# vaenyr/stable-diffusion-on-device

Measured on AMD Instinct MI355X. Metric: images/sec + per-UNet-step ms, SD v1.4 512x512 20-step PLMS, 1/2/4/8 MI355X, higher is better.
Workload: dtype f16

## Files before the change

stable-diffusion-on-device_amd/csrc/attention.hip:

```cpp
#include "common.h"
#include "sdod_hip.h"
#include "host_util.h"

#include <cstdlib>
#include <type_traits>

namespace {

struct AttnP {
    const f16* q;
    const f16* k;
    const f16* v;
    f16* out;
    int B, H, Lq, Lk;
    int ldq, ldk, ldv, ldo;
    float scale_log2;
    int causal;
};

typedef short short4v __attribute__((__vector_size__(4 * sizeof(short))));
typedef __attribute__((address_space(3))) short4v* lds_short4_ptr;

constexpr int odd16(int dv) {
    int s = (dv + 15) / 16;
    if ((s & 1) == 0) s += 1;
    return s * 16;
}

template <int D, int QT>
constexpr int attn_min_waves() { return (D == 40 || (D == 80 && QT == 1)) ? 3 : 1; }

template <int N, int I = 0, class F>
SDOD_DEVICE void static_for(F&& f) {
    if constexpr (I < N) {
        f(std::integral_constant<int, I>{});
        static_for<N, I + 1>(f);
    }
}

template <int D, int QT, bool TR, int KVS = 1>
__global__ __launch_bounds__(256 * KVS, (attn_min_waves<D, QT>())) void attn_kernel(const AttnP p) {
    constexpr int DP = ((D + 31) / 32) * 32;
    constexpr int KSTEPS = DP / 32;
    constexpr int DV = ((D + 15) / 16) * 16;
    constexpr int NDT = DV / 16;
    constexpr int KSTR = DP + 8;
    constexpr int VSTR = odd16(DV);
    constexpr int KT = 64;
    constexpr int DC = D / 8;
    constexpr int LD_IT = (KT * DC + 255) / 256;
    constexpr int STAGE = KT * (KSTR + VSTR);
    constexpr bool SUM_BY_MFMA = DV > D;
    static_assert(D % 8 == 0, "head dim must be a multiple of 8");

    extern __shared__ __attribute__((aligned(16))) char smem_raw[];
    const int grp = KVS > 1 ? (int)(threadIdx.x >> 8) : 0;
    f16* smem = reinterpret_cast<f16*>(smem_raw) + (size_t)grp * 2 * STAGE;

    const int tid = threadIdx.x & 255;
    const int lane = tid & 63;
    const int wave = tid >> 6;
    const int g = lane >> 4;
    const int li = lane & 15;
    const int nqb = (p.Lq + 64 * QT - 1) / (64 * QT);
    const int lid = xcd_remap(blockIdx.x, nqb * p.H * p.B);
    const int bh = lid / nqb;
    const int b = bh / p.H, h = bh - b * p.H;
    const int q_block = (lid - bh * nqb) * (64 * QT);

    const f16* kbase = p.k + (size_t)b * p.Lk * p.ldk + h * D;
    const f16* vbase = p.v + (size_t)b * p.Lk * p.ldv + h * D;

    {
        constexpr int KPADC = (DP - D) / 8, VPADC = (DV - D) / 8;
        for (int st = 0; st < 2; ++st) {
            f16* sK = smem + st * STAGE;
            f16* sV = sK + KT * KSTR;
            if (KPADC > 0)
                for (int idx = tid; idx < KT * KPADC; idx += 256) {
                    const int row = idx / (KPADC > 0 ? KPADC : 1), ch = idx - row * KPADC;
                    *reinterpret_cast<f16x8*>(sK + row * KSTR + D + ch * 8) = zero8();
                }
            if (VPADC > 0)
                for (int idx = tid; idx < KT * VPADC; idx += 256) {
                    const int row = idx / (VPADC > 0 ? VPADC : 1), ch = idx - row * VPADC;
                    f16x8 pad = zero8();
                    if (ch == 0) pad[0] = (f16)1.0f;
                    *reinterpret_cast<f16x8*>(sV + row * VSTR + D + ch * 8) = pad;
                }
        }
    }

    f16x8 qf[QT][KSTEPS];
    int qrow[QT];
#pragma unroll
    for (int t = 0; t < QT; ++t) {
        qrow[t] = q_block + wave * (16 * QT) + t * 16 + li;
        const f16* qp = p.q + ((size_t)b * p.Lq + qrow[t]) * p.ldq + h * D;
#pragma unroll
        for (int ks = 0; ks < KSTEPS; ++ks) {
            const int d0 = ks * 32 + g * 8;
            qf[t][ks] = (qrow[t] < p.Lq && d0 + 8 <= D) ? ldg8(qp + d0) : zero8();
        }
    }

    int kend = p.Lk;
    if (p.causal) kend = min(p.Lk, q_block + 64 * QT);
    const int NT = (kend + KT - 1) / KT;

    f16x8 rk[LD_IT], rv[LD_IT];
    const f16* kptr0[LD_IT];
    const f16* vptr0[LD_IT];
#pragma unroll
    for (int i = 0; i < LD_IT; ++i) {
        const int idx = tid + 256 * i;
        const int row = idx / DC, ch = idx - row * DC;
        kptr0[i] = kbase + (size_t)row * p.ldk + ch * 8;
        vptr0[i] = vbase + (size_t)row * p.ldv + ch * 8;
    }
    auto load_tile = [&](int t) {
        if (t * KT + KT <= p.Lk) {
            const size_t ko = (size_t)t * KT * p.ldk, vo = (size_t)t * KT * p.ldv;
#pragma unroll
            for (int i = 0; i < LD_IT; ++i) {
                if (tid + 256 * i < KT * DC) {
                    rk[i] = ldg8(kptr0[i] + ko);
                    rv[i] = ldg8(vptr0[i] + vo);
                }
            }
            return;
        }
#pragma unroll
        for (int i = 0; i < LD_IT; ++i) {
            const int idx = tid + 256 * i;
            const int row = idx / DC, ch = idx - row * DC;
            const int key = t * KT + row;
            const bool ok = (idx < KT * DC) && (key < p.Lk);
            rk[i] = ok ? ldg8(kbase + (size_t)key * p.ldk + ch * 8) : zero8();
            rv[i] = ok ? ldg8(vbase + (size_t)key * p.ldv + ch * 8) : zero8();
        }
    };
    auto store_tile = [&](int st) {
        f16* sK = smem + st * STAGE;
        f16* sV = sK + KT * KSTR;
#pragma unroll
        for (int i = 0; i < LD_IT; ++i) {
            const int idx = tid + 256 * i;
            const int row = idx / DC, ch = idx - row * DC;
            if (idx < KT * DC) {
                *reinterpret_cast<f16x8*>(sK + row * KSTR + ch * 8) = rk[i];
                *reinterpret_cast<f16x8*>(sV + row * VSTR + ch * 8) = rv[i];
            }
        }
    };

    f32x4 o[QT][NDT];
    float m_run[QT], l_run[QT];
#pragma unroll
    for (int t = 0; t < QT; ++t) {
        m_run[t] = -1e30f;
        l_run[t] = 0.f;
#pragma unroll
        for (int dt = 0; dt < NDT; ++dt) o[t][dt] = f32x4{0.f, 0.f, 0.f, 0.f};
    }

#ifdef SDOD_ATTN_ABLATE
    constexpr int abl = SDOD_ATTN_ABLATE;
#else
    constexpr int abl = 0;
#endif
    constexpr bool HOLD = D <= 80;
    auto read_vt = [&](const f16* sV, int u, int dt) -> f16x8 {
        const f16* a0 = sV + (32 * u + 4 * g + (li >> 2)) * VSTR + dt * 16 + 4 * (li & 3);
        const short4v lo = __builtin_amdgcn_ds_read_tr16_b64_v4i16((lds_short4_ptr)(a0));
        const short4v hi = __builtin_amdgcn_ds_read_tr16_b64_v4i16((lds_short4_ptr)(a0 + 16 * VSTR));
        typedef short short8v __attribute__((__vector_size__(8 * sizeof(short))));
        const short8v both = __builtin_shufflevector(lo, hi, 0, 1, 2, 3, 4, 5, 6, 7);
        return __builtin_bit_cast(f16x8, both);
    };
    auto softmax_pv = [&](auto a_c, int t, f32x4 (&s_a)[4], const f16x8 (&vfr)[HOLD ? 2 : 1][HOLD ? NDT : 1], const f16* sV) {
        constexpr int a = decltype(a_c)::value;
        const bool need_mask = (t * KT + KT > p.Lk) || (p.causal && (t * KT + KT - 1 > q_block + wave * (16 * QT)));
        if (need_mask) {
            int key0 = t * KT + g * 4;
            asm volatile("" : "+v"(key0));
#pragma unroll
            for (int c = 0; c < 4; ++c)
#pragma unroll
                for (int r = 0; r < 4; ++r) {
                    const int key = key0 + c * 16 + r;
                    const bool masked = (key >= p.Lk) | (p.causal & (key > qrow[a]));
                    s_a[c][r] = masked ? -1e30f : s_a[c][r];
                }
        }
        float mx;
        {
            const float t0 = fmaxf(fmaxf(s_a[0][0], s_a[0][1]), s_a[0][2]);
            const float t1 = fmaxf(fmaxf(s_a[0][3], s_a[1][0]), s_a[1][1]);
            const float t2 = fmaxf(fmaxf(s_a[1][2], s_a[1][3]), s_a[2][0]);
            const float t3 = fmaxf(fmaxf(s_a[2][1], s_a[2][2]), s_a[2][3]);
            const float t4 = fmaxf(fmaxf(s_a[3][0], s_a[3][1]), s_a[3][2]);
            const float u0 = fmaxf(fmaxf(t0, t1), t2);
            const float u1 = fmaxf(fmaxf(t3, t4), s_a[3][3]);
            mx = fmaxf(u0, u1);
        }
        mx = quad_rows_max(mx);
        const float m_new = fmaxf(m_run[a], mx * p.scale_log2);
        const bool rescale = __builtin_amdgcn_ballot_w64(m_new != m_run[a]) != 0;
        const float alpha = rescale ? __builtin_amdgcn_exp2f(m_run[a] - m_new) : 1.0f;
        m_run[a] = m_new;
        float rs[4] = {0.f, 0.f, 0.f, 0.f};
        const float sc = p.scale_log2, nm = -m_new;
#pragma unroll
        for (int c = 0; c < 4; ++c) {
#pragma unroll
            for (int r = 0; r < 4; ++r) {
                float v = __builtin_fmaf(s_a[c][r], sc, nm);
                if (!(abl & 2)) v = __builtin_amdgcn_exp2f(v);
                if (!SUM_BY_MFMA) rs[r] += v;
                s_a[c][r] = v;
            }
        }
        if (!SUM_BY_MFMA) l_run[a] = __builtin_fmaf(l_run[a], alpha, (rs[0] + rs[1]) + (rs[2] + rs[3]));
        if (rescale) {
#pragma unroll
            for (int dt = 0; dt < NDT; ++dt)
#pragma unroll
                for (int r = 0; r < 4; ++r) o[a][dt][r] *= alpha;
        }
        f16x8 pf[2];
#pragma unroll
        for (int u = 0; u < 2; ++u) {
            f16x8 f;
#pragma unroll
            for (int r = 0; r < 4; ++r) {
                f[r] = (f16)s_a[2 * u][r];
                f[4 + r] = (f16)s_a[2 * u + 1][r];
            }
            pf[u] = f;
        }
#pragma unroll
        for (int u = 0; u < 2; ++u) {
#pragma unroll
            for (int dt = 0; dt < NDT; ++dt) {
                f16x8 vf;
                if (TR) {
                    vf = HOLD ? vfr[u][dt] : read_vt(sV, u, dt);
                } else {
#pragma unroll
                    for (int e = 0; e < 8; ++e) vf[e] = sV[(32 * u + 16 * (e >> 2) + 4 * g + (e & 3)) * VSTR + dt * 16 + li];
                }
                o[a][dt] = mfma16(vf, pf[u], o[a][dt]);
            }
        }
    };
    auto read_k = [&](const f16* sK, f16x8 (&kf)[HOLD ? KSTEPS : 1][4]) {
        if constexpr (HOLD) {
#pragma unroll
            for (int ks = 0; ks < KSTEPS; ++ks)
#pragma unroll
                for (int c = 0; c < 4; ++c) kf[ks][c] = *reinterpret_cast<const f16x8*>(sK + (c * 16 + li) * KSTR + ks * 32 + g * 8);
        }
    };
    auto read_v = [&](const f16* sV, f16x8 (&vfr)[HOLD ? 2 : 1][HOLD ? NDT : 1]) {
        if constexpr (TR && HOLD) {
#pragma unroll
            for (int u = 0; u < 2; ++u)
#pragma unroll
                for (int dt = 0; dt < NDT; ++dt) vfr[u][dt] = read_vt(sV, u, dt);
        }
    };
    auto qk = [&](const f16* sK, const f16x8 (&kf)[HOLD ? KSTEPS : 1][4], f32x4 (&s)[QT][4]) {
#pragma unroll
        for (int a = 0; a < QT; ++a) {
#pragma unroll
            for (int c = 0; c < 4; ++c) s[a][c] = f32x4{0.f, 0.f, 0.f, 0.f};
#pragma unroll
            for (int ks = 0; ks < KSTEPS; ++ks)
#pragma unroll
                for (int c = 0; c < 4; ++c) {
                    const f16x8 k8 = HOLD ? kf[ks][c] : *reinterpret_cast<const f16x8*>(sK + (c * 16 + li) * KSTR + ks * 32 + g * 8);
                    s[a][c] = mfma16(k8, qf[a][ks], s[a][c]);
                }
        }
    };

    if (grp < NT) {
        load_tile(grp);
        store_tile(0);
    }
    __syncthreads();
    const int NTG = (NT + KVS - 1) / KVS;
    for (int it = 0; it < NTG; ++it) {
        const int t = it * KVS + grp;
        const int cur = it & 1;
        const bool has_next = t + KVS < NT;
        const f16* sK = smem + cur * STAGE;
        const f16* sV = sK + KT * KSTR;
        if (t >= NT) {
            __syncthreads();
            continue;
        }
        f16x8 kf[HOLD ? KSTEPS : 1][4];
        f16x8 vfr[HOLD ? 2 : 1][HOLD ? NDT : 1];
        read_k(sK, kf);
        read_v(sV, vfr);
        f32x4 s[QT][4];
        qk(sK, kf, s);
        if (has_next && !(abl & 1)) load_tile(t + KVS);
        static_for<QT>([&](auto a_c) { softmax_pv(a_c, t, s[decltype(a_c)::value], vfr, sV); });
        if (has_next) store_tile(cur ^ 1);
        __syncthreads();
    }

    if constexpr (KVS > 1) {
        static_assert(KVS == 2, "the merge below handles two groups");
        float* mrg = reinterpret_cast<float*>(smem_raw);
        constexpr int NV = QT * (2 + NDT * 4);
        static_assert((size_t)NV * 256 * sizeof(float) <= (size_t)KVS * 2 * STAGE * sizeof(f16), "merge buffer fits the staging LDS");
        if (grp == 1) {
#pragma unroll
            for (int a = 0; a < QT; ++a) {
                mrg[(a * (2 + NDT * 4) + 0) * 256 + tid] = m_run[a];
                mrg[(a * (2 + NDT * 4) + 1) * 256 + tid] = l_run[a];
#pragma unroll
                for (int dt = 0; dt < NDT; ++dt)
#pragma unroll
                    for (int r = 0; r < 4; ++r) mrg[(a * (2 + NDT * 4) + 2 + dt * 4 + r) * 256 + tid] = o[a][dt][r];
            }
        }
        __syncthreads();
        if (grp == 1) return;
#pragma unroll
        for (int a = 0; a < QT; ++a) {
            const float m1 = mrg[(a * (2 + NDT * 4) + 0) * 256 + tid], l1 = mrg[(a * (2 + NDT * 4) + 1) * 256 + tid];
            const float m = fmaxf(m_run[a], m1);
            const float a0 = __builtin_amdgcn_exp2f(m_run[a] - m), a1 = __builtin_amdgcn_exp2f(m1 - m);
            l_run[a] = l_run[a] * a0 + l1 * a1;
#pragma unroll
            for (int dt = 0; dt < NDT; ++dt)
#pragma unroll
                for (int r = 0; r < 4; ++r) o[a][dt][r] = o[a][dt][r] * a0 + mrg[(a * (2 + NDT * 4) + 2 + dt * 4 + r) * 256 + tid] * a1;
            m_run[a] = m;
        }
    }
#pragma unroll
    for (int a = 0; a < QT; ++a) {
        float l;
        if (SUM_BY_MFMA) {
            l = __shfl(o[a][D / 16][D % 4], ((D % 16) / 4) * 16 + li);
        } else {
            l = quad_rows_sum(l_run[a]);
        }
        const float inv = l > 0.f ? 1.0f / l : 0.f;
        if (qrow[a] < p.Lq) {
            f16* op = p.out + ((size_t)b * p.Lq + qrow[a]) * p.ldo + h * D;
#pragma unroll
            for (int dt = 0; dt < NDT; ++dt) {
                const int dv0 = dt * 16 + g * 4;
                if (dv0 < D) {
                    f16x4 hv;
#pragma unroll
                    for (int r = 0; r < 4; ++r) hv[r] = (f16)(o[a][dt][r] * inv);
                    *reinterpret_cast<f16x4*>(op + dv0) = hv;
                }
            }
        }
    }
}

template <int D, int QT, bool TR, int KVS = 1>
hipError_t attn_launch(const AttnP& p, hipStream_t st) {
    constexpr int DP = ((D + 31) / 32) * 32;
    constexpr int DV = ((D + 15) / 16) * 16;
    constexpr size_t smem = (size_t)KVS * 2 * 64 * (DP + 8 + odd16(DV)) * sizeof(f16);
    static_assert(smem <= 160 * 1024, "LDS");
    static std::atomic<unsigned long long> attr_devs{0};
    if (sdod::first_use_on_device(attr_devs)) {
        hipError_t e = hipFuncSetAttribute(reinterpret_cast<const void*>(&attn_kernel<D, QT, TR, KVS>),
                                           hipFuncAttributeMaxDynamicSharedMemorySize, (int)smem);
        if (e != hipSuccess) return e;
    }
    dim3 grid(((p.Lq + 64 * QT - 1) / (64 * QT)) * p.H * p.B);
    SDOD_LAUNCH((attn_kernel<D, QT, TR, KVS>), grid, dim3(256 * KVS), smem, st, p);
    return hipGetLastError();
}

template <int D>
hipError_t attn_dispatch(const AttnP& p, bool big, bool tr, hipStream_t st) {
    if (tr) return big ? attn_launch<D, 2, true>(p, st) : attn_launch<D, 1, true>(p, st);
    return big ? attn_launch<D, 2, false>(p, st) : attn_launch<D, 1, false>(p, st);
}

struct FoldP {
    const f16* kv; int ld_kv, k_off, v_off, L, n_img;
    const f16* wq; int ldq;
    const float* sq; const float* tq;
    const f16* wo; int ldwo;
    int heads, d, C;
    float alpha;
    f16* w1; float* s1; float* t1; f16* w2;
    int tiles_c;
    int n_w;
};
constexpr int kFoldKMax = 160;
__global__ __launch_bounds__(256) void xattn_fold_kernel(const FoldP p) {
    __shared__ __attribute__((aligned(16))) f16 sa[80][kFoldKMax + 8], sb[80][kFoldKMax + 8];
    const int tid = threadIdx.x, lane = tid & 63, wave = tid >> 6;
    const int NK = p.heads * 80, d = p.d;
    int item = blockIdx.x;
    if (item >= 2 * p.n_w) {
        const int idx = (item - 2 * p.n_w) * 256 + tid;
        if (idx >= p.n_img * NK) return;
        const int j = idx % 80, bh = idx / 80, h = bh % p.heads, img = bh / p.heads;
        if (j >= p.L) {
            p.s1[idx] = 0.f;
            p.t1[idx] = -30000.f;
            return;
        }
        const f16* kr = p.kv + ((long long)img * p.L + j) * p.ld_kv + p.k_off + h * d;
        float a = 0.f, b = 0.f;
        for (int dd = 0; dd < d; ++dd) {
            const float kval = (float)kr[dd];
            a = fmaf(kval, p.sq[h * d + dd], a);
            b = fmaf(kval, p.tq[h * d + dd], b);
        }
        p.s1[idx] = p.alpha * a;
        p.t1[idx] = p.alpha * b;
        return;
    }
    const bool second = item >= p.n_w;
    if (second) item -= p.n_w;
    const int tc = item % p.tiles_c, bh = item / p.tiles_c, h = bh % p.heads, img = bh / p.heads;
    const int KP = (d + 31) & ~31, kc = KP / 8;
    auto stage_rows = [&](f16 (*dst)[kFoldKMax + 8], const f16* base, long long row_stride, int valid_rows) {
        for (int idx = tid; idx < 80 * kc; idx += 256) {
            const int r = idx / kc, ch = idx - r * kc;
            const f16x8 v = (r < valid_rows && ch * 8 < d) ? ldg8(base + (long long)r * row_stride + ch * 8) : zero8();
            *reinterpret_cast<f16x8*>(&dst[r][ch * 8]) = v;
        }
    };
    if (!second) {
        stage_rows(sa, p.kv + (long long)img * p.L * p.ld_kv + p.k_off + h * d, p.ld_kv, p.L);
        for (int idx = tid; idx < KP * 10; idx += 256) {
            const int k = idx / 10, ch = idx - k * 10;
            const f16x8 v = k < d ? ldg8(p.wq + (long long)(h * d + k) * p.ldq + tc * 80 + ch * 8) : zero8();
#pragma unroll
            for (int e = 0; e < 8; ++e) sb[ch * 8 + e][k] = v[e];
        }
    } else {
        stage_rows(sa, p.wo + (long long)(tc * 80) * p.ldwo + h * d, p.ldwo, 80);
        stage_rows(sb, p.kv + (long long)img * p.L * p.ld_kv + p.v_off + h * d, p.ld_kv, p.L);
    }
    __syncthreads();
    const int fr = lane & 15, fg = lane >> 4;
    for (int rb = wave; rb < 5; rb += 4) {
        f32x4 acc[5];
#pragma unroll
        for (int j = 0; j < 5; ++j) acc[j] = f32x4{0.f, 0.f, 0.f, 0.f};
        for (int ks = 0; ks < KP / 32; ++ks) {
            const f16x8 fa = *reinterpret_cast<const f16x8*>(&sa[rb * 16 + fr][ks * 32 + fg * 8]);
#pragma unroll
            for (int j = 0; j < 5; ++j) {
                const f16x8 fb = *reinterpret_cast<const f16x8*>(&sb[j * 16 + fr][ks * 32 + fg * 8]);
                acc[j] = mfma16(fb, fa, acc[j]);
            }
        }
        const int m = rb * 16 + fr;
        f16* row = second ? p.w2 + ((long long)img * p.C + tc * 80 + m) * NK + h * 80
                          : p.w1 + ((long long)(img * p.heads + h) * 80 + m) * p.C + tc * 80;
        const float al = second ? 1.0f : p.alpha;
#pragma unroll
        for (int j = 0; j < 5; ++j) {
            f16x4 o;
#pragma unroll
            for (int r = 0; r < 4; ++r) o[r] = (f16)(al * acc[j][r]);
            *reinterpret_cast<f16x4*>(row + j * 16 + fg * 4) = o;
        }
    }
}

}

extern "C" int sdod_attention_f16(const void* q, const void* k, const void* v, void* out, int batch, int heads, int lq,
                                  int lk, int d, int ldq, int ldk, int ldv, int ldo, float scale, int causal,
                                  void* stream) {
    SDOD_TRY
    SDOD_REQUIRE(q && k && v && out, "null pointer");
    SDOD_REQUIRE(batch > 0 && heads > 0 && lq > 0 && lk > 0, "bad shape");
    SDOD_REQUIRE(d == 40 || d == 64 || d == 80 || d == 160, "head dim must be one of 40, 64, 80, 160");
    SDOD_REQUIRE(ldq % 8 == 0 && ldk % 8 == 0 && ldv % 8 == 0 && ldo % 4 == 0, "row strides must keep 16-byte alignment");
    SDOD_REQUIRE(ldq >= heads * d && ldk >= heads * d && ldv >= heads * d && ldo >= heads * d, "row stride < heads*d");
    SDOD_REQUIRE((((uintptr_t)q | (uintptr_t)k | (uintptr_t)v) & 15) == 0 && ((uintptr_t)out & 7) == 0, "misaligned pointer");
    AttnP p{};
    p.q = (const f16*)q; p.k = (const f16*)k; p.v = (const f16*)v; p.out = (f16*)out;
    p.B = batch; p.H = heads; p.Lq = lq; p.Lk = lk;
    p.ldq = ldq; p.ldk = ldk; p.ldv = ldv; p.ldo = ldo;
    p.scale_log2 = scale * 1.4426950408889634f;
    p.causal = causal;
    const bool no_tr = std::getenv("SDOD_ATTN_NO_TR") != nullptr;
    const bool tr = !no_tr;
    bool big = lq >= 2048 && d != 160;
    if (const char* e = std::getenv("SDOD_ATTN_QT")) big = e[0] == '2' && d != 160;
    hipStream_t st = (hipStream_t)stream;
    hipError_t e;
    switch (d) {
    case 40: e = attn_dispatch<40>(p, big, tr, st); break;
    case 64: e = attn_dispatch<64>(p, big, tr, st); break;
    case 80: {
        static const bool kvs_off = [] { const char* e2 = std::getenv("SDOD_ATTN_KVS"); return e2 && e2[0] == '0'; }();
        const long long wgs = (long long)((lq + 63) / 64) * heads * batch;
        if (!big && tr && !kvs_off && !causal && wgs <= 512 && lk >= 256) e = attn_launch<80, 1, true, 2>(p, st);
        else e = attn_dispatch<80>(p, big, tr, st);
        break;
    }
    default: e = attn_dispatch<160>(p, false, tr, st); break;
    }
    SDOD_HIP_CHECK(e);
    return 0;
    SDOD_CATCH
}

extern "C" int sdod_xattn_fold_f16(const void* kv, int ld_kv, int k_off, int v_off, int n_img, int L, const void* wq, int ldq,
                                   const void* sq, const void* tq, const void* wo, int ldwo, int heads, int d, float scale, void* w1,
                                   void* s1, void* t1, void* w2, void* stream) {
    SDOD_TRY
    SDOD_REQUIRE(kv && wq && sq && tq && wo && w1 && s1 && t1 && w2, "null pointer");
    SDOD_REQUIRE(n_img > 0 && heads > 0 && d > 0 && d <= kFoldKMax && d % 8 == 0 && L > 0 && L <= 80, "bad shape (d <= 160, d % 8 == 0, L <= 80)");
    const int C = heads * d, NK = heads * 80;
    SDOD_REQUIRE(C % 80 == 0 && ldq >= C && ldwo >= C && ld_kv >= C, "heads * d must be a multiple of 80; row strides >= heads * d");
    SDOD_REQUIRE(ld_kv % 8 == 0 && k_off % 8 == 0 && v_off % 8 == 0 && ldq % 8 == 0 && ldwo % 8 == 0 &&
                     (((uintptr_t)kv | (uintptr_t)wq | (uintptr_t)wo | (uintptr_t)w1 | (uintptr_t)w2) & 15) == 0,
                 "operands must keep 16-byte alignment");
    FoldP p{};
    p.kv = (const f16*)kv; p.ld_kv = ld_kv; p.k_off = k_off; p.v_off = v_off; p.L = L; p.n_img = n_img;
    p.wq = (const f16*)wq; p.ldq = ldq; p.sq = (const float*)sq; p.tq = (const float*)tq;
    p.wo = (const f16*)wo; p.ldwo = ldwo;
    p.heads = heads; p.d = d; p.C = C;
    p.alpha = scale * 1.4426950408889634f;
    p.w1 = (f16*)w1; p.s1 = (float*)s1; p.t1 = (float*)t1; p.w2 = (f16*)w2;
    p.tiles_c = C / 80;
    p.n_w = n_img * heads * p.tiles_c;
    const int blocks = 2 * p.n_w + (n_img * NK + 255) / 256;
    SDOD_LAUNCH(xattn_fold_kernel, dim3(blocks), dim3(256), 0, (hipStream_t)stream, p);
    SDOD_HIP_CHECK(hipGetLastError());
    return 0;
    SDOD_CATCH
}
```

Baseline: 10.42.

## Use lazy threshold-based max rescaling in flash attention softmax

Changes the online softmax so the running max is set on the first tile and afterwards updated only when some lane's new score exceeds it by more than a threshold (default 8, env-configurable). Scores are pre-scaled and shifted by the running max with inline fma/max3 assembly, which skips the cross-lane max reduction, the exp of alpha and the rescaling of the output accumulators on most tiles. Launch bounds for the split-KV variant now request KVS waves minimum. The trade is that unnormalized probabilities can reach up to 2^thr before fp16 conversion, which narrows precision headroom.

```diff
diff --git a/stable-diffusion-on-device_amd/csrc/attention.hip b/stable-diffusion-on-device_amd/csrc/attention.hip
--- a/stable-diffusion-on-device_amd/csrc/attention.hip
+++ b/stable-diffusion-on-device_amd/csrc/attention.hip
@@ -15,6 +15,7 @@
     int B, H, Lq, Lk;
     int ldq, ldk, ldv, ldo;
     float scale_log2;
+    float thr;
     int causal;
 };
 
@@ -27,8 +28,8 @@
     return s * 16;
 }
 
-template <int D, int QT>
-constexpr int attn_min_waves() { return (D == 40 || (D == 80 && QT == 1)) ? 3 : 1; }
+template <int D, int QT, int KVS>
+constexpr int attn_min_waves() { return KVS > 1 ? KVS : (D == 40 || (D == 80 && QT == 1)) ? 3 : 1; }
 
 template <int N, int I = 0, class F>
 SDOD_DEVICE void static_for(F&& f) {
@@ -39,7 +40,7 @@
 }
 
 template <int D, int QT, bool TR, int KVS = 1>
-__global__ __launch_bounds__(256 * KVS, (attn_min_waves<D, QT>())) void attn_kernel(const AttnP p) {
+__global__ __launch_bounds__(256 * KVS, (attn_min_waves<D, QT, KVS>())) void attn_kernel(const AttnP p) {
     constexpr int DP = ((D + 31) / 32) * 32;
     constexpr int KSTEPS = DP / 32;
     constexpr int DV = ((D + 15) / 16) * 16;
@@ -158,7 +159,7 @@
     float m_run[QT], l_run[QT];
 #pragma unroll
     for (int t = 0; t < QT; ++t) {
-        m_run[t] = -1e30f;
+        m_run[t] = 0.f;
         l_run[t] = 0.f;
 #pragma unroll
         for (int dt = 0; dt < NDT; ++dt) o[t][dt] = f32x4{0.f, 0.f, 0.f, 0.f};
@@ -178,7 +179,8 @@
         const short8v both = __builtin_shufflevector(lo, hi, 0, 1, 2, 3, 4, 5, 6, 7);
         return __builtin_bit_cast(f16x8, both);
     };
-    auto softmax_pv = [&](auto a_c, int t, f32x4 (&s_a)[4], const f16x8 (&vfr)[HOLD ? 2 : 1][HOLD ? NDT : 1], const f16* sV) {
+    auto softmax_pv = [&](auto a_c, int t, bool first, f32x4 (&s_a)[4], const f16x8 (&vfr)[HOLD ? 2 : 1][HOLD ? NDT : 1],
+                          const f16* sV) {
         constexpr int a = decltype(a_c)::value;
         const bool need_mask = (t * KT + KT > p.Lk) || (p.causal && (t * KT + KT - 1 > q_block + wave * (16 * QT)));
         if (need_mask) {
@@ -193,41 +195,50 @@
                     s_a[c][r] = masked ? -1e30f : s_a[c][r];
                 }
         }
-        float mx;
-        {
-            const float t0 = fmaxf(fmaxf(s_a[0][0], s_a[0][1]), s_a[0][2]);
-            const float t1 = fmaxf(fmaxf(s_a[0][3], s_a[1][0]), s_a[1][1]);
-            const float t2 = fmaxf(fmaxf(s_a[1][2], s_a[1][3]), s_a[2][0]);
-            const float t3 = fmaxf(fmaxf(s_a[2][1], s_a[2][2]), s_a[2][3]);
-            const float t4 = fmaxf(fmaxf(s_a[3][0], s_a[3][1]), s_a[3][2]);
-            const float u0 = fmaxf(fmaxf(t0, t1), t2);
-            const float u1 = fmaxf(fmaxf(t3, t4), s_a[3][3]);
-            mx = fmaxf(u0, u1);
-        }
-        mx = quad_rows_max(mx);
-        const float m_new = fmaxf(m_run[a], mx * p.scale_log2);
-        const bool rescale = __builtin_amdgcn_ballot_w64(m_new != m_run[a]) != 0;
-        const float alpha = rescale ? __builtin_amdgcn_exp2f(m_run[a] - m_new) : 1.0f;
-        m_run[a] = m_new;
+        const float sc = p.scale_log2, nm = -m_run[a];
+#pragma unroll
+        for (int c = 0; c < 4; ++c)
+#pragma unroll
+            for (int r = 0; r < 4; ++r) asm("v_fma_f32 %0, %1, %2, %3" : "=v"(s_a[c][r]) : "v"(s_a[c][r]), "s"(sc), "v"(nm));
+        auto max3 = [](float x, float y, float z) {
+            float r;
+            asm("v_max3_f32 %0, %1, %2, %3" : "=v"(r) : "v"(x), "v"(y), "v"(z));
+            return r;
+        };
+        const float u0 = max3(max3(s_a[0][0], s_a[0][1], s_a[0][2]), max3(s_a[0][3], s_a[1][0], s_a[1][1]),
+                              max3(s_a[1][2], s_a[1][3], s_a[2][0]));
+        const float u1 = max3(max3(s_a[2][1], s_a[2][2], s_a[2][3]), max3(s_a[3][0], s_a[3][1], s_a[3][2]), s_a[3][3]);
+        const float mx = max3(u0, u1, u1);
+        if (first || __builtin_amdgcn_ballot_w64(mx > p.thr) != 0) {
+            float mxq = mx;
+            asm volatile("" : "+v"(mxq));
+            const float dm = first ? quad_rows_max(mxq) : fmaxf(quad_rows_max(mxq), 0.f);
+            m_run[a] += dm;
+            if (!first) {
+                const float alpha = __builtin_amdgcn_exp2f(-dm);
+                if (!SUM_BY_MFMA) l_run[a] *= alpha;
+#pragma unroll
+                for (int dt = 0; dt < NDT; ++dt)
+#pragma unroll
+                    for (int r = 0; r < 4; ++r) o[a][dt][r] *= alpha;
+            }
+#pragma unroll
+            for (int c = 0; c < 4; ++c)
+#pragma unroll
+                for (int r = 0; r < 4; ++r) s_a[c][r] -= dm;
+        }
         float rs[4] = {0.f, 0.f, 0.f, 0.f};
-        const float sc = p.scale_log2, nm = -m_new;
 #pragma unroll
         for (int c = 0; c < 4; ++c) {
 #pragma unroll
             for (int r = 0; r < 4; ++r) {
-                float v = __builtin_fmaf(s_a[c][r], sc, nm);
+                float v = s_a[c][r];
                 if (!(abl & 2)) v = __builtin_amdgcn_exp2f(v);
                 if (!SUM_BY_MFMA) rs[r] += v;
                 s_a[c][r] = v;
             }
         }
-        if (!SUM_BY_MFMA) l_run[a] = __builtin_fmaf(l_run[a], alpha, (rs[0] + rs[1]) + (rs[2] + rs[3]));
-        if (rescale) {
-#pragma unroll
-            for (int dt = 0; dt < NDT; ++dt)
-#pragma unroll
-                for (int r = 0; r < 4; ++r) o[a][dt][r] *= alpha;
-        }
+        if (!SUM_BY_MFMA) l_run[a] += (rs[0] + rs[1]) + (rs[2] + rs[3]);
         f16x8 pf[2];
 #pragma unroll
         for (int u = 0; u < 2; ++u) {
@@ -291,6 +302,7 @@
     }
     __syncthreads();
     const int NTG = (NT + KVS - 1) / KVS;
+    int first = 1;
     for (int it = 0; it < NTG; ++it) {
         const int t = it * KVS + grp;
         const int cur = it & 1;
@@ -308,8 +320,10 @@
         f32x4 s[QT][4];
         qk(sK, kf, s);
         if (has_next && !(abl & 1)) load_tile(t + KVS);
-        static_for<QT>([&](auto a_c) { softmax_pv(a_c, t, s[decltype(a_c)::value], vfr, sV); });
+        static_for<QT>([&](auto a_c) { softmax_pv(a_c, t, first != 0, s[decltype(a_c)::value], vfr, sV); });
         if (has_next) store_tile(cur ^ 1);
+        first = 0;
+        asm volatile("" : "+s"(first));
         __syncthreads();
     }
 
@@ -321,7 +335,7 @@
         if (grp == 1) {
 #pragma unroll
             for (int a = 0; a < QT; ++a) {
-                mrg[(a * (2 + NDT * 4) + 0) * 256 + tid] = m_run[a];
+                mrg[(a * (2 + NDT * 4) + 0) * 256 + tid] = first ? -1e30f : m_run[a];
                 mrg[(a * (2 + NDT * 4) + 1) * 256 + tid] = l_run[a];
 #pragma unroll
                 for (int dt = 0; dt < NDT; ++dt)
@@ -497,6 +511,9 @@
     p.B = batch; p.H = heads; p.Lq = lq; p.Lk = lk;
     p.ldq = ldq; p.ldk = ldk; p.ldv = ldv; p.ldo = ldo;
     p.scale_log2 = scale * 1.4426950408889634f;
+    p.thr = 8.0f;
+    if (const char* e = std::getenv("SDOD_ATTN_THR")) p.thr = std::strtof(e, nullptr);
+    SDOD_REQUIRE(p.thr >= 0.f && p.thr <= 14.f, "SDOD_ATTN_THR must lie in [0, 14] (P <= 2^thr is rounded to fp16)");
     p.causal = causal;
     const bool no_tr = std::getenv("SDOD_ATTN_NO_TR") != nullptr;
     const bool tr = !no_tr;
```

Result: no change. 10.51, median of 6 (+0.8%).
